# ericehanley/gke-ray-train

Measured on AMD Instinct MI355X. Metric: tokens/sec (whole node) Llama-2-7B fine-tune at 1/2/4/8 MI355X; samples/sec on Wikitext-2, higher is better.
Workload: dtype bf16; 1 GPU; model=llama2-7b, global_batch=8, seq_len=1024, parallelism=dp1, micro_batch=8, grad_accum=1, optimizer=fused AdamW fp32 states, activation_checkpointing=False, optimizer_overlap=True, forced_collectives=False, library_gemms=offline-tuned

## Files before the change

### gke_ray_train_amd/csrc/bindings/ops.cpp

```cpp
#include <climits>
#include <torch/extension.h>

#include <algorithm>
#include <cmath>
#include <c10/hip/HIPStream.h>
#include <c10/core/DeviceGuard.h>

#include "grt_kernels.h"
#include "grt_sdma.h"

namespace {

using at::Tensor;
using c10::optional;

hipStream_t cur_stream(const Tensor& t) {
  return c10::hip::getCurrentHIPStream(t.device().index()).stream();
}

grt::DType dtype_of(const Tensor& t) {
  if (t.scalar_type() == at::kBFloat16) return grt::DType::BF16;
  TORCH_CHECK(t.scalar_type() == at::kFloat, "gke_ray_train_amd kernels support bf16/fp32, got ", t.scalar_type());
  return grt::DType::F32;
}
// ... 1619 lines not shown
  m.def("lora_down", &lora_down, py::arg("x"), py::arg("a"), py::arg("p"), py::arg("seed"), py::arg("offset"),
        py::arg("want_xd"), py::arg("h_out") = py::none(), py::arg("hscale") = 1.0);
  m.def("lora_dx", &lora_dx, py::arg("g"), py::arg("at"), py::arg("dx"), py::arg("p"), py::arg("seed"),
        py::arg("offset"), py::arg("accumulate"), py::arg("dx_in") = py::none(), py::arg("gscale") = 1.0);
  m.def("lora_refresh", &lora_refresh, py::arg("bs"), py::arg("offs"), py::arg("w"), py::arg("wt"), py::arg("col0"),
        py::arg("wt_row0") = -1);
  m.def("lora_g", &lora_g, py::arg("a"), py::arg("bt"), py::arg("c"), py::arg("alpha"), py::arg("accumulate"));
  m.def("lora_g_group", &lora_g_group, py::arg("a"), py::arg("bt"), py::arg("c"), py::arg("alpha"),
        py::arg("accumulate"));
  m.def("lora_tred", &lora_tred, py::arg("a"), py::arg("h"), py::arg("out"), py::arg("alpha"), py::arg("accumulate"),
        py::arg("transpose"));
  m.def("lora_tred_group", &lora_tred_group, py::arg("a"), py::arg("h"), py::arg("out"), py::arg("alpha"),
        py::arg("accumulate"));
  m.def("dropout_bwd_seeded", &dropout_bwd_seeded);
  m.def("ce_fwd", &ce_fwd);
  m.def("ce_bwd", &ce_bwd);
  m.def("sumsq_blocks", &sumsq_blocks);
  m.def("lds_fill", [](int64_t pattern, int64_t device) {
    c10::OptionalDeviceGuard g(c10::Device(c10::DeviceType::CUDA, (c10::DeviceIndex)device));
    grt::lds_fill((uint32_t)pattern, c10::hip::getCurrentHIPStream((c10::DeviceIndex)device).stream());
  }, "test support: fill every CU's LDS with a 32-bit pattern (stale-LDS-read detection)");
  m.def("sumsq", &sumsq);
  m.def("clip_finalize", &clip_finalize);
  m.def("adamw", &adamw, py::arg("p"), py::arg("g"), py::arg("m"), py::arg("v"), py::arg("master"),
        py::arg("hyper"), py::arg("gscale"), py::arg("max_blocks") = 0, py::arg("index_offset") = 0);
  m.def("adamw_t", &adamw_t);
  m.def("adamw8", &adamw8, py::arg("p"), py::arg("g"), py::arg("codes_m"), py::arg("absmax_m"), py::arg("codes_v"),
        py::arg("absmax_v"), py::arg("master"), py::arg("hyper"), py::arg("gscale"), py::arg("max_blocks") = 0,
        py::arg("index_offset") = 0);
  m.def("quantize_blockwise8", &quantize_blockwise8, py::arg("x"), py::arg("codes"), py::arg("absmax"),
        py::arg("signed"));
  m.def("dequantize_blockwise8", &dequantize_blockwise8, py::arg("codes"), py::arg("absmax"), py::arg("out"),
        py::arg("signed"));
  m.def("scale_", &scale_);
  m.def("attn_fwd", &attn_fwd, py::arg("q"), py::arg("k"), py::arg("v"), py::arg("out"), py::arg("scale"),
        py::arg("causal"), py::arg("seqlens_k"), py::arg("dropout_p") = 0.0, py::arg("seed") = 0,
        py::arg("cu_seqlens") = py::none(), py::arg("max_seqlen") = 0, py::arg("o_t") = py::none());
  m.def("attn_bwd", &attn_bwd, py::arg("dout"), py::arg("q"), py::arg("k"), py::arg("v"), py::arg("o"),
        py::arg("lse"), py::arg("dq"), py::arg("dk"), py::arg("dv"), py::arg("scale"), py::arg("causal"),
        py::arg("seqlens_k"), py::arg("dropout_p") = 0.0, py::arg("seed") = 0, py::arg("rope_cos") = py::none(),
        py::arg("rope_sin") = py::none(), py::arg("cu_seqlens") = py::none(), py::arg("max_seqlen") = 0,
        py::arg("dqkv_t") = py::none());
  m.def("rope_attn_fwd_d64", &rope_attn_fwd_d64, py::arg("qkv"), py::arg("cos"), py::arg("sin"), py::arg("o"),
        py::arg("B"), py::arg("S"), py::arg("hq"), py::arg("hkv"), py::arg("scale"), py::arg("causal"),
        py::arg("cu_seqlens") = py::none(), py::arg("max_seqlen") = 0,
        "bf16 head_dim 64: RoPE + flash attention straight from the fused QKV rows (packed with cu_seqlens) -> lse");
  m.def("rope_attn_bwd_d64", &rope_attn_bwd_d64, py::arg("do"), py::arg("qkv"), py::arg("cos"), py::arg("sin"),
        py::arg("o"), py::arg("lse"), py::arg("dqkv"), py::arg("B"), py::arg("S"), py::arg("hq"), py::arg("hkv"),
        py::arg("scale"), py::arg("causal"), py::arg("cu_seqlens") = py::none(), py::arg("max_seqlen") = 0,
        "backward of rope_attn_fwd_d64: un-rotated dQ / dK and dV into the columns of dqkv (every element written)");
  m.def("attn_set_schedule", &grt::attn_set_schedule,
        "bf16 attention causal-pair / XCD-grouped schedule, bit mask: 1 = forward, 2 = dQ, 4 = dK/dV");
  m.def("attn_get_schedule", &grt::attn_get_schedule);
  m.def("attn_set_dkdv_form", &grt::attn_set_dkdv_form, "dK / dV kernel: 1 = 4-wave, 2 = wave-pair (default)");
  m.def("attn_get_dkdv_form", &grt::attn_get_dkdv_form);
  m.def("attn_set_dma_fast", &grt::attn_set_dma_fast, "1 = hoisted LDS-DMA addressing (default), 0 = clamped per tile");
  m.def("ew_set_fast", &grt::ew_set_fast, "1 = single-pass RoPE (D = 128) / SwiGLU kernels (default), 0 = grid-stride kernels");
  m.def("attn_set_skip_dead", &grt::attn_set_skip_dead,
        "1 = forward / dK-dV waves skip the causal tiles they mask entirely (default), 0 = compute them");
  m.def("nf4_quantize", &nf4_quantize);
  m.def("nf4_dequantize", &nf4_dequantize);
  m.def("nf4_dequantize_t", &nf4_dequantize_t);
  m.def("nf4_dequantize_into", &nf4_dequantize_into);
  m.def("rmsnorm_bwd_dx", &rmsnorm_bwd_dx);
  m.def("swiglu_fwd_t", &swiglu_fwd_t);
  m.def("swiglu_bwd_t", &swiglu_bwd_t);
  m.def("transpose_into", &transpose_into);
  m.def("copy_sdma", &copy_sdma);
  m.def("sdma_d2h", &sdma_d2h, py::arg("dst"), py::arg("src"), py::arg("producer_stream") = 0,
        "pinned host <- device on an SDMA engine, ordered on the source's current stream; producer_stream "
        "(a raw stream handle): the stream whose work so far wrote src");
  m.def("sdma_stats", &sdma_stats, "copies / bytes / worker busy seconds / first error of the SDMA copier");
  m.def("sdma_clear_error", [](int64_t device) { grt::sdma_clear_error((int)device); });
  m.def("gemv", &gemv, py::arg("x"), py::arg("w"), py::arg("swiglu") = false);
  m.def("gemv_fused", &gemv_fused, py::arg("x"), py::arg("w"), py::arg("sumsq"), py::arg("slot"),
        py::arg("swiglu") = false, py::arg("g") = py::none(), py::arg("res") = py::none(), py::arg("eps") = 1e-5,
        py::arg("cos") = py::none(), py::arg("sin") = py::none(), py::arg("pos") = py::none(),
        py::arg("kc") = py::none(), py::arg("vc") = py::none(), py::arg("hq") = 0, py::arg("hkv") = 0);
  m.def("nf4_gemv", &nf4_gemv, py::arg("x"), py::arg("qweight"), py::arg("absmax"), py::arg("N"), py::arg("K"),
        py::arg("h") = py::none(), py::arg("lora_b") = py::none(), py::arg("lora_off") = py::none(),
        py::arg("scaling") = 1.0);
  m.def("sample_logits", &sample_logits, py::arg("logits"), py::arg("do_sample") = false, py::arg("temperature") = 1.0,
        py::arg("top_k") = 0, py::arg("top_p") = 1.0, py::arg("seed") = 0, py::arg("counter") = py::none(),
        py::arg("keep_mask") = py::none(), py::arg("finished") = py::none(), py::arg("finish_step") = py::none(),
        py::arg("step") = py::none(), py::arg("next_ids") = py::none(), py::arg("out") = py::none(),
        py::arg("eos_ids") = py::none(), py::arg("pad_id") = py::none(), py::arg("max_steps") = 1);
  m.def("attn_decode", &attn_decode);
  m.def("attn_decode_d64", &attn_decode_d64);
  m.def("attn_decode_d64_partials", &attn_decode_d64_partials,
        "test support: attn_decode_d64 and its per-split (o, max, sum) partial states");
  m.def("embedding_fwd", &embedding_fwd);
  m.def("embedding_bwd", &embedding_bwd);
  m.def("gemm_wgrad", &gemm_wgrad, py::arg("x"), py::arg("y"), py::arg("out"), py::arg("accumulate"),
        py::arg("mode") = 0);
  m.def("gemm_supported", &gemm_supported, py::arg("a"), py::arg("b"), py::arg("out"));
  m.def("gemm_nt", &gemm_nt, py::arg("a"), py::arg("b"), py::arg("out"), py::arg("accumulate") = false,
        py::arg("variant") = 0);
  m.def("gemm_wgrad2", &gemm_wgrad2, py::arg("x"), py::arg("y"), py::arg("out"), py::arg("accumulate") = false);
  m.def("gemm_nn", &gemm_nn, py::arg("a"), py::arg("b"), py::arg("out"), py::arg("accumulate") = false);
  m.def("ipc_alloc", &ipc_alloc);
  m.def("ipc_free", &ipc_free_ptr);
  m.def("ipc_handle", &ipc_handle);
  m.def("ipc_open", &ipc_open);
  m.def("ipc_close", &ipc_close);
  m.def("ipc_allreduce", &ipc_allreduce);
  m.def("ipc_barrier", &ipc_barrier);
  m.def("cu_masked_stream", &cu_masked_stream);
// ... 5 lines not shown
```

### gke_ray_train_amd/csrc/kernels/attention.hip

```cpp
#include <limits.h>
#include <stdlib.h>

#include <type_traits>
#include <utility>

#include "grt_attn_dropout.h"
#include "grt_common.h"
#include "grt_kernels.h"
#include "grt_lds_image.h"
#include "grt_mfma.h"

namespace grt {
namespace {

using namespace lds_image;

constexpr int D = 128;
constexpr int kChunks = D / 8;

__device__ __forceinline__ bf16x8 lds_row_read(const char* base, int row, int ch) {
  return *reinterpret_cast<const bf16x8*>(base + chunk_off(row, ch));
}

constexpr float kLog2e = 1.4426950408889634f;
constexpr float kLn2 = 0.6931471805599453f;

__device__ __forceinline__ float halves_max(float x) {
  const auto r = __builtin_amdgcn_permlane32_swap(__float_as_uint(x), __float_as_uint(x), false, false);
  return fmaxf(__uint_as_float(r[0]), __uint_as_float(r[1]));
}

constexpr float kDeferLog2 = 8.f;

template <class F, int... I>
__device__ __forceinline__ void static_for(F&& f, std::integer_sequence<int, I...>) {
  (f(std::integral_constant<int, I>{}), ...);
}
__device__ __forceinline__ void wait_tiles4(int tiles) {
  if (tiles >= 4) asm volatile("s_waitcnt vmcnt(16)" ::: "memory");
  else if (tiles == 3) asm volatile("s_waitcnt vmcnt(12)" ::: "memory");
  else if (tiles == 2) asm volatile("s_waitcnt vmcnt(8)" ::: "memory");
  else if (tiles == 1) asm volatile("s_waitcnt vmcnt(4)" ::: "memory");
  else asm volatile("s_waitcnt vmcnt(0)" ::: "memory");
}

constexpr int F3M = 128, F3N = 32, F3NT = 256, F3NSLOT = 4;
constexpr int F3IMG = F3N * D * 2;
constexpr int F3SLOT = 2 * F3IMG;

struct QJobs {
  int bh;
  int blk0, blk1;
};
__device__ __forceinline__ QJobs q_jobs(int sched, int nqb, int BH) {
  QJobs j;
  if (sched == 1) {
    const int npair = (nqb + 1) >> 1, nwg = BH * npair;
    const int bid = blockIdx.x, xcd = bid & 7, q8 = nwg >> 3, r8 = nwg & 7;
    const int L = (xcd < r8 ? xcd * (q8 + 1) : r8 * (q8 + 1) + (xcd - r8) * q8) + (bid >> 3);
    j.bh = L / npair;
    const int pr = L % npair;
    j.blk0 = nqb - 1 - pr;
    j.blk1 = pr != nqb - 1 - pr ? pr : -1;
  } else {
    j.bh = blockIdx.x % BH;
    j.blk0 = nqb - 1 - (int)(blockIdx.x / BH);
    j.blk1 = -1;
  }
  return j;
}
__host__ __device__ inline unsigned q_grid(int sched, int nqb, int BH) {
  return (unsigned)(sched == 1 ? BH * ((nqb + 1) / 2) : BH * nqb);
}

template <bool DROP, int NS>
__global__ __launch_bounds__(F3NT, 2) void attn_fwd_kernel(const AttnParams p) {
  __shared__ __attribute__((aligned(16))) char smem[NS * F3SLOT];
  const int tid = threadIdx.x, lane = tid & 63, h = lane >> 5, l32 = lane & 31;
  const int w = __builtin_amdgcn_readfirstlane(tid >> 6);
  const int g = lane >> 4, l16 = lane & 15;
  const int nqb = (p.Sq + F3M - 1) / F3M;
  const int BH = p.B * p.Hq;
  const QJobs jobs = q_jobs(p.sched, nqb, BH);
  const int bh = jobs.bh;
  const int b = bh / p.Hq, hq = bh % p.Hq;
  const int hkv = hq / (p.Hq / p.Hkv);
  GRT_DEVICE_CHECK(b < p.B && hkv < p.Hkv && jobs.blk0 >= 0 && jobs.blk0 < nqb);
  auto run_block = [&](const int qblk) {
  int Sq = p.Sq, Sk = p.Sk;
  int64_t tok0 = 0;
  if (p.cu_seqlens) {
    tok0 = p.cu_seqlens[b];
    Sq = Sk = p.cu_seqlens[b + 1] - (int)tok0;
    if (qblk * F3M >= Sq) return;
  }
  const int sk = p.seqlens_k ? min(Sk, p.seqlens_k[b]) : Sk;
  const int off = Sk - Sq;
  const int q0 = qblk * F3M, qw0 = q0 + w * 32;
  const int myq = qw0 + l32;

  const bf16* Q = (const bf16*)p.q + (int64_t)b * p.q_bs + tok0 * p.q_ss + (int64_t)hq * p.q_hs;
  const bf16* K = (const bf16*)p.k + (int64_t)b * p.k_bs + tok0 * p.k_ss + (int64_t)hkv * p.k_hs;
  const bf16* Vg = (const bf16*)p.v + (int64_t)b * p.v_bs + tok0 * p.v_ss + (int64_t)hkv * p.v_hs;

  bf16x8 qf[D / 16];
#pragma unroll
  for (int ks = 0; ks < D / 16; ++ks) {
    if (myq < Sq) qf[ks] = *reinterpret_cast<const bf16x8*>(Q + (int64_t)myq * p.q_ss + ks * 16 + 8 * h);
    else qf[ks] = bf16x8{};
  }
  const int klim = p.causal ? min(sk - 1, myq + off) : sk - 1;
  const int kmask = p.causal ? min(sk, qw0 + off + 1) : sk;
  const int klast = p.skip_dead && p.causal ? min(sk - 1, qw0 + 31 + off) : INT_MAX;

  int kend = sk;
  if (p.causal) kend = min(kend, q0 + F3M + off);
  const int nt = kend > 0 ? (kend + F3N - 1) / F3N : 0;

  const uint32_t smem0 = lds_addr(smem);
  const int row0 = 8 * w + g, row1 = row0 + 4;
  const int ch0 = l16 ^ swz(row0), ch1 = l16 ^ swz(row1);
  const uint32_t ko0 = (uint32_t)(row0 * p.k_ss + ch0 * 8), ko1 = (uint32_t)(row1 * p.k_ss + ch1 * 8);
  const uint32_t vo0 = (uint32_t)(row0 * p.v_ss + ch0 * 8), vo1 = (uint32_t)(row1 * p.v_ss + ch1 * 8);
  auto dma_tile = [&](int t, uint32_t slot_off) {
    const uint32_t dst = __builtin_amdgcn_readfirstlane(smem0 + slot_off + (uint32_t)(8 * w * 256));
    if (p.dma_fast && (t + 1) * F3N <= Sk) {
// ... 118 lines not shown
    for (; t + UNR <= ntl; t += UNR) static_for([&](auto i_c) { step_i(t, i_c); }, std::make_integer_sequence<int, UNR>{});
    static_for([&](auto i_c) { if (t + decltype(i_c)::value < ntl) step_i(t, i_c); }, std::make_integer_sequence<int, UNR - 1>{});
    for (t = ntl; t < nt; ++t) {
      asm volatile("s_waitcnt lgkmcnt(0)" ::: "memory");
      if (t + 1 < nt) wait_dma(min(nt, t + NS - 1) - (t + 2));
      __builtin_amdgcn_s_barrier();
      if (t + NS - 1 < nt) dma_tile(t + NS - 1, (uint32_t)(((t + NS - 1) % NS) * F3SLOT));
    }
  }
  asm volatile("s_waitcnt vmcnt(0)" ::: "memory");

  const float lt = l + __shfl_xor(l, 32, 64);
  const float inv = lt > 0.f ? 1.f / lt : 0.f;
  bf16* O = (bf16*)p.o + (int64_t)b * p.o_bs + (tok0 + min(myq, Sq - 1)) * p.o_ss + (int64_t)hq * p.o_hs;
#pragma unroll
  for (int db = 0; db < 4; ++db)
#pragma unroll
    for (int gp = 0; gp < 2; ++gp) {
      union { bf16x4 v; uint32_t u[2]; } a, c2;
#pragma unroll
      for (int j = 0; j < 4; ++j) {
        a.v[j] = static_cast<bf16>(o[db][8 * gp + j] * inv);
        c2.v[j] = static_cast<bf16>(o[db][8 * gp + 4 + j] * inv);
      }
      const auto r0 = __builtin_amdgcn_permlane32_swap(a.u[0], c2.u[0], false, false);
      const auto r1 = __builtin_amdgcn_permlane32_swap(a.u[1], c2.u[1], false, false);
      if (myq < Sq) {
        *reinterpret_cast<uint4*>(O + db * 32 + 16 * gp + 8 * h) = make_uint4(r0[0], r1[0], r0[1], r1[1]);
        if (p.o_t != nullptr) {
          bf16* ot = static_cast<bf16*>(p.o_t) + (int64_t)(hq * D) * p.ot_ld + (p.cu_seqlens ? 0 : (int64_t)b * p.Sq) +
                     tok0 + myq;
          const int d0 = db * 32 + 8 * (2 * gp) + 4 * h, d1 = db * 32 + 8 * (2 * gp + 1) + 4 * h;
#pragma unroll
          for (int j = 0; j < 4; ++j) {
            ot[(int64_t)(d0 + j) * p.ot_ld] = a.v[j];
            ot[(int64_t)(d1 + j) * p.ot_ld] = c2.v[j];
          }
        }
      }
    }
  if (myq < Sq) {
    if (h == 0 && p.lse)
      p.lse[((int64_t)b * p.Hq + hq) * p.Sq + myq] = lt > 0.f ? (m + __log2f(lt)) * kLn2 : INFINITY;
  }
  };
  run_block(jobs.blk0);
  if (jobs.blk1 >= 0) {
    asm volatile("s_waitcnt lgkmcnt(0)" ::: "memory");
    __builtin_amdgcn_s_barrier();
    run_block(jobs.blk1);
  }
}

__host__ __device__ inline int sq_pad(int Sq) { return (Sq + 31) / 32 * 32; }

__global__ __launch_bounds__(256) void attn_bwd_pre_kernel(const AttnBwdParams p) {
  const int l16 = threadIdx.x & 15;
  const int Sqp = sq_pad(p.f.Sq);
  const int64_t row = (int64_t)blockIdx.x * 16 + (threadIdx.x >> 4);
  const int64_t nrows = (int64_t)p.f.B * p.f.Hq * Sqp;
  if (row >= nrows) return;
  const int q = (int)(row % Sqp);
  const int64_t bh = row / Sqp;
  float acc = 0.f;
  const int hq = (int)(bh % p.f.Hq), b = (int)(bh / p.f.Hq);
  int Sq = p.f.Sq;
  int64_t tok0 = 0;
  if (p.f.cu_seqlens) {
    tok0 = p.f.cu_seqlens[b];
    Sq = p.f.cu_seqlens[b + 1] - (int)tok0;
  }
  if (q < Sq) {
    const bf16* O = (const bf16*)p.f.o + (int64_t)b * p.f.o_bs + (int64_t)hq * p.f.o_hs + (tok0 + q) * p.f.o_ss;
    const bf16* dO = (const bf16*)p.dout + (int64_t)b * p.do_bs + (int64_t)hq * p.do_hs + (tok0 + q) * p.do_ss;
    float a[8], g[8];
    load16(O + l16 * 8, a);
    load16(dO + l16 * 8, g);
#pragma unroll
    for (int k = 0; k < 8; ++k) acc += a[k] * g[k];
  }
#pragma unroll
  for (int o = 8; o >= 1; o >>= 1) acc += __shfl_xor(acc, o, 16);
  if (l16 == 0) {
    float* lse2 = p.delta + nrows;
    p.delta[row] = acc;
    lse2[row] = q < Sq ? p.f.lse[bh * p.f.Sq + q] * kLog2e : INFINITY;
  }
}


struct TCopy {
  bf16* p;
  int64_t ld;
};
__device__ __forceinline__ void st_t(const TCopy& tc, int d, const bf16x4& v) {
  if (tc.p != nullptr) {
#pragma unroll
    for (int j = 0; j < 4; ++j) tc.p[(int64_t)(d + j) * tc.ld] = v[j];
  }
}
__device__ __forceinline__ TCopy tcopy(const AttnBwdParams& P, int row0, int head, int64_t tok) {
  if (P.dqkv_t == nullptr) return TCopy{nullptr, 0};
  return TCopy{static_cast<bf16*>(P.dqkv_t) + (int64_t)(row0 + head * D) * P.t_ld + tok, P.t_ld};
}

__device__ __forceinline__ void store_unrotated(const f32x16 (&acc)[4], float scale, const float* __restrict__ cr,
                                                const float* __restrict__ sr, bf16* dst, int h,
                                                const TCopy& tc = TCopy{nullptr, 0}) {
#pragma unroll
  for (int db = 0; db < 2; ++db)
#pragma unroll
    for (int gg = 0; gg < 4; ++gg) {
      const int d = db * 32 + 8 * gg + 4 * h;
      const f32x4 c = *reinterpret_cast<const f32x4*>(cr + d);
      const f32x4 sn = *reinterpret_cast<const f32x4*>(sr + d);
      bf16x4 lo, hi;
#pragma unroll
      for (int j = 0; j < 4; ++j) {
        const float x1 = acc[db][4 * gg + j] * scale, x2 = acc[db + 2][4 * gg + j] * scale;
        lo[j] = static_cast<bf16>(x1 * c[j] + x2 * sn[j]);
        hi[j] = static_cast<bf16>(x2 * c[j] - x1 * sn[j]);
      }
      *reinterpret_cast<bf16x4*>(dst + d) = lo;
      *reinterpret_cast<bf16x4*>(dst + d + D / 2) = hi;
      st_t(tc, d, lo);
      st_t(tc, d + D / 2, hi);
    }
}

constexpr int K2N = 128, K2M = 32, K2NT = 256, K2NSLOT = 4;
constexpr int K2IMG = K2M * D * 2;
constexpr int K2SLOT = 2 * K2IMG + 4 * 1024;

template <bool DROP>
__global__ __launch_bounds__(K2NT, 1) void attn_bwd_dkdv_kernel(const AttnBwdParams P) {
  const AttnParams& p = P.f;
  __shared__ __attribute__((aligned(16))) char smem[K2NSLOT * K2SLOT];
  const int tid = threadIdx.x, lane = tid & 63, h = lane >> 5, l32 = lane & 31;
  const int w = __builtin_amdgcn_readfirstlane(tid >> 6);
  const int g = lane >> 4, l16 = lane & 15;
  const int BHk = p.B * p.Hkv;
  const int nkb = (p.Sk + K2N - 1) / K2N;
  QJobs jobs;
  if (p.sched == 1) {
    jobs = q_jobs(1, nkb, BHk);
  } else {
    jobs.bh = blockIdx.x % BHk;
    jobs.blk0 = (int)(blockIdx.x / BHk);
    jobs.blk1 = -1;
  }
  const int bhk = jobs.bh;
  const int b = bhk / p.Hkv, hkv = bhk % p.Hkv;
  const int grp = p.Hq / p.Hkv;
  auto run_block = [&](const int kblk) {
  int Sq = p.Sq, Sk = p.Sk;
  int64_t tok0 = 0;
  if (p.cu_seqlens) {
    tok0 = p.cu_seqlens[b];
    Sq = Sk = p.cu_seqlens[b + 1] - (int)tok0;
    if (kblk * K2N >= Sk) return;
  }
  GRT_DEVICE_CHECK(grp * p.Hkv == p.Hq && kblk * K2N < Sk);
  const int sk = p.seqlens_k ? min(Sk, p.seqlens_k[b]) : Sk;
  const int off = Sk - Sq;
  const int k0 = kblk * K2N, kw0 = k0 + w * 32, mykey = kw0 + l32;
  const float c = p.scale * kLog2e;
  const int Sqp = sq_pad(p.Sq);
  const float* lse2 = P.delta + (int64_t)p.B * p.Hq * Sqp;

  const bf16* K = (const bf16*)p.k + (int64_t)b * p.k_bs + tok0 * p.k_ss + (int64_t)hkv * p.k_hs;
  const bf16* Vg = (const bf16*)p.v + (int64_t)b * p.v_bs + tok0 * p.v_ss + (int64_t)hkv * p.v_hs;
  bf16x8 kf[D / 16], vf[D / 16];
#pragma unroll
  for (int ks = 0; ks < D / 16; ++ks) {
    if (mykey < sk) {
      kf[ks] = *reinterpret_cast<const bf16x8*>(K + (int64_t)mykey * p.k_ss + ks * 16 + 8 * h);
      vf[ks] = *reinterpret_cast<const bf16x8*>(Vg + (int64_t)mykey * p.v_ss + ks * 16 + 8 * h);
    } else {
      kf[ks] = bf16x8{};
      vf[ks] = bf16x8{};
    }
// ... 363 lines not shown
      bf16x8 fq[D / 16];
#pragma unroll
      for (int ks = 0; ks < D / 16; ++ks) fq[ks] = lds_row_read(qi, l32, 2 * ks + h);
#pragma unroll
      for (int ks = 0; ks < D / 16; ++ks) s = mfma32(fq[ks], kv[ks], s);
      __builtin_amdgcn_sched_barrier(0);
      float* xo = xbase + (t & 1) * (K3X / 4);
#pragma unroll
      for (int q = 0; q < 4; ++q) {
        const f32x4 ls = *reinterpret_cast<const f32x4*>(st + 8 * q + 4 * h);
        f32x4 pv;
#pragma unroll
        for (int j = 0; j < 4; ++j) pv[j] = fast_exp2(fmaf(s[4 * q + j], c, -ls[j]));
        *reinterpret_cast<f32x4*>(xo + (q * 64 + lane) * 4) = pv;
#pragma unroll
        for (int j = 0; j < 4; ++j) s[4 * q + j] = pv[j];
      }
      const bf16x8 pb0 = pack8(s, 0), pb1 = pack8(s, 8);
      __builtin_amdgcn_sched_barrier(0);
#pragma unroll
      for (int stp = 0; stp < 2; ++stp) {
        const int kk = 16 * stp + 4 * h;
#pragma unroll
        for (int db = 0; db < 4; ++db) {
          const int c0 = db * 32 + (g & 1) * 16;
          const bf16x8 a = cat(tr_read(qi + K3IMG, kk, c0, l16), tr_read(qi + K3IMG, kk + 8, c0, l16));
          acc[db] = mfma32(a, stp ? pb1 : pb0, acc[db]);
        }
      }
     }
    } else {
      if (t > 0 && !dead_p) finish(t - 1, smem + ((SL + K3NS - 1) % K3NS) * K3SLOT);
      __builtin_amdgcn_sched_barrier(0);
      if (!dead_c) {
        bf16x8 fd[D / 16];
#pragma unroll
        for (int ks = 0; ks < D / 16; ++ks) fd[ks] = lds_row_read(qi + K3IMG, l32, 2 * ks + h);
        dpc = f32x16{};
#pragma unroll
        for (int ks = 0; ks < D / 16; ++ks) dpc = mfma32(fd[ks], kv[ks], dpc);
      }
    }
    prv_h = cur_h;
    prv_q = cur_q;
    advance(cur_h, cur_q);
  };

  if (total > 0) {
    const int pre = min(total, K3PD);
    for (int j = 0; j < pre; ++j) {
      dma_tile(hkv * grp + dma_h, dma_q, (uint32_t)(j * K3SLOT));
      advance(dma_h, dma_q);
    }
    using I0 = std::integral_constant<int, 0>;
    using I1 = std::integral_constant<int, 1>;
    using I2 = std::integral_constant<int, 2>;
    using I3 = std::integral_constant<int, 3>;
    using I4 = std::integral_constant<int, 4>;
    int t = 0;
    for (; t + K3NS <= total; t += K3NS) {
      step(t, I0{});
      step(t + 1, I1{});
      step(t + 2, I2{});
      step(t + 3, I3{});
      step(t + 4, I4{});
    }
    if (t < total) step(t, I0{});
    if (t + 1 < total) step(t + 1, I1{});
    if (t + 2 < total) step(t + 2, I2{});
    if (t + 3 < total) step(t + 3, I3{});
    asm volatile("s_waitcnt lgkmcnt(0)" ::: "memory");
    __builtin_amdgcn_s_barrier();
    if constexpr (!SW) {
      if (prv_q + K3M > dead_q) finish(total - 1, smem + ((total - 1) % K3NS) * K3SLOT);
    }
  }
  asm volatile("s_waitcnt vmcnt(0)" ::: "memory");

  if (mykey < Sk) {
    const int64_t tokg = (p.cu_seqlens ? 0 : (int64_t)b * p.Sk) + tok0 + mykey;
    if constexpr (SW) {
      bf16* dV = (bf16*)P.dv + (int64_t)b * P.dv_bs + (int64_t)hkv * P.dv_hs + (tok0 + mykey) * P.dv_ss;
      const TCopy tv = tcopy(P, P.t_row_v, hkv, tokg);
#pragma unroll
      for (int db = 0; db < 4; ++db)
#pragma unroll
        for (int gg = 0; gg < 4; ++gg) {
          bf16x4 v;
#pragma unroll
          for (int j = 0; j < 4; ++j) v[j] = static_cast<bf16>(acc[db][4 * gg + j]);
          *reinterpret_cast<bf16x4*>(dV + db * 32 + 8 * gg + 4 * h) = v;
          st_t(tv, db * 32 + 8 * gg + 4 * h, v);
        }
    } else {
      bf16* dK = (bf16*)P.dk + (int64_t)b * P.dk_bs + (int64_t)hkv * P.dk_hs + (tok0 + mykey) * P.dk_ss;
      const TCopy tk = tcopy(P, P.t_row_k, hkv, tokg);
      if (P.rope_cos) {
        store_unrotated(acc, p.scale, P.rope_cos + (int64_t)mykey * (D / 2), P.rope_sin + (int64_t)mykey * (D / 2), dK, h,
                        tk);
      } else {
#pragma unroll
        for (int db = 0; db < 4; ++db)
#pragma unroll
          for (int gg = 0; gg < 4; ++gg) {
            bf16x4 a;
#pragma unroll
// ... 160 lines not shown
  };

  if (nt > 0) {
    const int pre = min(nt, Q2NSLOT - 1);
    for (int t = 0; t < pre; ++t) dma_tile(t, (uint32_t)(t * Q2SLOT));
    wait_dma(pre - 1);
    __builtin_amdgcn_s_barrier();
    f32x16 sA, dpA, sB, dpB;
    sdp(0, I0{}, sA, dpA);
    int t = 0;
    for (; t + Q2NSLOT <= nt; t += Q2NSLOT) {
      step(t, I0{}, sA, dpA, sB, dpB);
      step(t + 1, std::integral_constant<int, 1>{}, sB, dpB, sA, dpA);
      step(t + 2, std::integral_constant<int, 2>{}, sA, dpA, sB, dpB);
      step(t + 3, std::integral_constant<int, 3>{}, sB, dpB, sA, dpA);
    }
    if (t < nt) step(t, I0{}, sA, dpA, sB, dpB);
    if (t + 1 < nt) step(t + 1, std::integral_constant<int, 1>{}, sB, dpB, sA, dpA);
    if (t + 2 < nt) step(t + 2, std::integral_constant<int, 2>{}, sA, dpA, sB, dpB);
  }
  asm volatile("s_waitcnt vmcnt(0)" ::: "memory");

  if (qok) {
    bf16* dQ = (bf16*)P.dq + (int64_t)b * P.dq_bs + (int64_t)hq * P.dq_hs + (tok0 + myq) * P.dq_ss;
    const TCopy tq = tcopy(P, P.t_row_q, hq, (p.cu_seqlens ? 0 : (int64_t)b * p.Sq) + tok0 + myq);
    if (P.rope_cos) {
      store_unrotated(dq, p.scale, P.rope_cos + (int64_t)myq * (D / 2), P.rope_sin + (int64_t)myq * (D / 2), dQ, h, tq);
    } else {
#pragma unroll
      for (int db = 0; db < 4; ++db)
#pragma unroll
        for (int gg = 0; gg < 4; ++gg) {
          bf16x4 v;
#pragma unroll
          for (int j = 0; j < 4; ++j) v[j] = static_cast<bf16>(dq[db][4 * gg + j] * p.scale);
          *reinterpret_cast<bf16x4*>(dQ + db * 32 + 8 * gg + 4 * h) = v;
          st_t(tq, db * 32 + 8 * gg + 4 * h, v);
        }
    }
  }
  };
  run_block(jobs.blk0);
  if (jobs.blk1 >= 0) {
    asm volatile("s_waitcnt lgkmcnt(0)" ::: "memory");
    __builtin_amdgcn_s_barrier();
    run_block(jobs.blk1);
  }
}

}

namespace {
int g_sched = 7;
int g_dkdv = 2;
int g_skip_dead = -1;
int skip_dead_now() {
  if (g_skip_dead < 0) {
    const char* e = getenv("GRT_ATTN_SKIP");
    g_skip_dead = e && atoi(e) == 0 ? 0 : 1;
  }
  return g_skip_dead;
}
int g_dma_fast = 1;
int dma_fast_for(const AttnParams& p, int64_t do_ss) {
  const int64_t lim = (int64_t)1 << 24;
  return g_dma_fast && p.q_ss < lim && p.k_ss < lim && p.v_ss < lim && do_ss < lim && p.q_ss >= 0 &&
         p.k_ss >= 0 && p.v_ss >= 0 && do_ss >= 0;
}
}

static int cu_count() {
  static const int n = [] {
    int d = 0, c = 256;
    hipGetDevice(&d);
    hipDeviceGetAttribute(&c, hipDeviceAttributeMultiprocessorCount, d);
    return c > 0 ? c : 256;
  }();
  return n;
}
static int pair_if_fills(int want, int nblk, int groups, int per_cu) {
  return want && (int64_t)groups * ((nblk + 1) / 2) >= (int64_t)cu_count() * per_cu ? 1 : 0;
}

void attn_set_schedule(int s) { g_sched = s; }
void attn_set_dkdv_form(int f) { g_dkdv = f == 1 ? 1 : 2; }
int attn_get_dkdv_form() { return g_dkdv; }
void attn_set_dma_fast(int on) { g_dma_fast = on ? 1 : 0; }
void attn_set_skip_dead(int on) { g_skip_dead = on ? 1 : 0; }
int attn_get_schedule() { return g_sched; }

static int sched_for(const AttnParams& p, int bit) { return p.cu_seqlens ? 0 : (g_sched >> bit) & 1; }

void attn_fwd(const AttnParams& p0, hipStream_t s) {
  AttnParams p = p0;
  p.dma_fast = dma_fast_for(p, 0);
  p.skip_dead = skip_dead_now();
  const int nqb = (p.Sq + F3M - 1) / F3M;
  p.sched = pair_if_fills(sched_for(p, 0), nqb, p.B * p.Hq, 2);
  const dim3 grid(q_grid(p.sched, nqb, p.B * p.Hq));
  if (p.drop_thresh) hipLaunchKernelGGL((attn_fwd_kernel<true, F3NSLOT>), grid, dim3(F3NT), 0, s, p);
  else hipLaunchKernelGGL((attn_fwd_kernel<false, F3NSLOT>), grid, dim3(F3NT), 0, s, p);
}

int64_t attn_bwd_workspace_floats(int B, int Hq, int Sq, int Dh) {
  (void)Dh;
  return 2 * (int64_t)B * Hq * sq_pad(Sq);
}

void attn_bwd(const AttnBwdParams& p0, hipStream_t s) {
  AttnBwdParams p = p0;
  p.f.dma_fast = dma_fast_for(p.f, p.do_ss);
  p.f.skip_dead = skip_dead_now();
  const int64_t rows = (int64_t)p.f.B * p.f.Hq * sq_pad(p.f.Sq);
  hipLaunchKernelGGL(attn_bwd_pre_kernel, dim3((unsigned)((rows + 15) / 16)), dim3(256), 0, s, p);
  const int nkb = (p.f.Sk + K2N - 1) / K2N;
  const int nqb = (p.f.Sq + Q2M - 1) / Q2M;
  AttnBwdParams pk = p, pq = p;
  pk.f.sched = pair_if_fills(sched_for(p.f, 2), nkb, p.f.B * p.f.Hkv, 1);
  pq.f.sched = pair_if_fills(sched_for(p.f, 1), nqb, p.f.B * p.f.Hq, 2);
  const dim3 g1(q_grid(pk.f.sched, nkb, p.f.B * p.f.Hkv)), g2(q_grid(pq.f.sched, nqb, p.f.B * p.f.Hq));
  static_assert(K3N == K2N, "both dK / dV forms take 128-key blocks (same grid)");
  if (p.f.drop_thresh) {
    hipLaunchKernelGGL(attn_bwd_dkdv_kernel<true>, g1, dim3(K2NT), 0, s, pk);
    hipLaunchKernelGGL(attn_bwd_dq_kernel<true>, g2, dim3(Q2NT), 0, s, pq);
  } else {
    if (g_dkdv == 2) hipLaunchKernelGGL(attn_bwd_dkdv2_kernel, g1, dim3(K3NT), 0, s, pk);
    else hipLaunchKernelGGL(attn_bwd_dkdv_kernel<false>, g1, dim3(K2NT), 0, s, pk);
    hipLaunchKernelGGL(attn_bwd_dq_kernel<false>, g2, dim3(Q2NT), 0, s, pq);
  }
}

}
```

Baseline: 28390 tokens/s.

## Add 256-key dK/dV attention backward kernel with 64 keys per wave pair

Adds a new dK/dV backward kernel in which each 512-thread workgroup handles 256 keys, split into four wave pairs of 64 keys. One wave of each pair computes the P/dV path and the other computes the dP/dK path, with a five-slot LDS pipeline for Q/dO tiles. The launcher picks it by default when there is no GQA, no packing, and the grid covers the CUs. This amortizes Q/dO tile loads over more keys per workgroup. The cost is one workgroup per CU and more registers; it also moves shared helpers into a header and adds a waitcnt in the existing kernel prologue.

```diff
diff --git a/gke_ray_train_amd/csrc/bindings/ops.cpp b/gke_ray_train_amd/csrc/bindings/ops.cpp
--- a/gke_ray_train_amd/csrc/bindings/ops.cpp
+++ b/gke_ray_train_amd/csrc/bindings/ops.cpp
@@ -1695,7 +1695,7 @@
   m.def("attn_set_schedule", &grt::attn_set_schedule,
         "bf16 attention causal-pair / XCD-grouped schedule, bit mask: 1 = forward, 2 = dQ, 4 = dK/dV");
   m.def("attn_get_schedule", &grt::attn_get_schedule);
-  m.def("attn_set_dkdv_form", &grt::attn_set_dkdv_form, "dK / dV kernel: 1 = 4-wave, 2 = wave-pair (default)");
+  m.def("attn_set_dkdv_form", &grt::attn_set_dkdv_form, "dK / dV kernel: 0 = chosen per launch (default), 1 = 4-wave, 2 = wave-pair, 32 keys per pair, 3 = wave-pair, 64 keys per pair");
   m.def("attn_get_dkdv_form", &grt::attn_get_dkdv_form);
   m.def("attn_set_dma_fast", &grt::attn_set_dma_fast, "1 = hoisted LDS-DMA addressing (default), 0 = clamped per tile");
   m.def("ew_set_fast", &grt::ew_set_fast, "1 = single-pass RoPE (D = 128) / SwiGLU kernels (default), 0 = grid-stride kernels");
diff --git a/gke_ray_train_amd/csrc/include/grt_attn_bwd.h b/gke_ray_train_amd/csrc/include/grt_attn_bwd.h
--- /dev/null
+++ b/gke_ray_train_amd/csrc/include/grt_attn_bwd.h
@@ -0,0 +1,90 @@
+#pragma once
+#include <hip/hip_runtime.h>
+
+#include "grt_common.h"
+#include "grt_kernels.h"
+#include "grt_lds_image.h"
+#include "grt_mfma.h"
+
+namespace grt {
+namespace attn128 {
+
+constexpr int D = 128;
+constexpr float kLog2e = 1.4426950408889634f;
+
+__device__ __forceinline__ bf16x8 lds_row_read(const char* base, int row, int ch) {
+  return *reinterpret_cast<const bf16x8*>(base + lds_image::chunk_off(row, ch));
+}
+
+struct QJobs {
+  int bh;
+  int blk0, blk1;
+};
+__device__ __forceinline__ QJobs q_jobs(int sched, int nqb, int BH) {
+  QJobs j;
+  if (sched == 1) {
+    const int npair = (nqb + 1) >> 1, nwg = BH * npair;
+    const int bid = blockIdx.x, xcd = bid & 7, q8 = nwg >> 3, r8 = nwg & 7;
+    const int L = (xcd < r8 ? xcd * (q8 + 1) : r8 * (q8 + 1) + (xcd - r8) * q8) + (bid >> 3);
+    j.bh = L / npair;
+    const int pr = L % npair;
+    j.blk0 = nqb - 1 - pr;
+    j.blk1 = pr != nqb - 1 - pr ? pr : -1;
+  } else {
+    j.bh = blockIdx.x % BH;
+    j.blk0 = nqb - 1 - (int)(blockIdx.x / BH);
+    j.blk1 = -1;
+  }
+  return j;
+}
+__host__ __device__ inline unsigned q_grid(int sched, int nqb, int BH) {
+  return (unsigned)(sched == 1 ? BH * ((nqb + 1) / 2) : BH * nqb);
+}
+
+__host__ __device__ inline int sq_pad(int Sq) { return (Sq + 31) / 32 * 32; }
+
+struct TCopy {
+  bf16* p;
+  int64_t ld;
+};
+__device__ __forceinline__ void st_t(const TCopy& tc, int d, const bf16x4& v) {
+  if (tc.p != nullptr) {
+#pragma unroll
+    for (int j = 0; j < 4; ++j) tc.p[(int64_t)(d + j) * tc.ld] = v[j];
+  }
+}
+__device__ __forceinline__ TCopy tcopy(const AttnBwdParams& P, int row0, int head, int64_t tok) {
+  if (P.dqkv_t == nullptr) return TCopy{nullptr, 0};
+  return TCopy{static_cast<bf16*>(P.dqkv_t) + (int64_t)(row0 + head * D) * P.t_ld + tok, P.t_ld};
+}
+
+__device__ __forceinline__ void store_unrotated(const f32x16 (&acc)[4], float scale, const float* __restrict__ cr,
+                                                const float* __restrict__ sr, bf16* dst, int h,
+                                                const TCopy& tc = TCopy{nullptr, 0}) {
+#pragma unroll
+  for (int db = 0; db < 2; ++db)
+#pragma unroll
+    for (int gg = 0; gg < 4; ++gg) {
+      const int d = db * 32 + 8 * gg + 4 * h;
+      const f32x4 c = *reinterpret_cast<const f32x4*>(cr + d);
+      const f32x4 sn = *reinterpret_cast<const f32x4*>(sr + d);
+      bf16x4 lo, hi;
+#pragma unroll
+      for (int j = 0; j < 4; ++j) {
+        const float x1 = acc[db][4 * gg + j] * scale, x2 = acc[db + 2][4 * gg + j] * scale;
+        lo[j] = static_cast<bf16>(x1 * c[j] + x2 * sn[j]);
+        hi[j] = static_cast<bf16>(x2 * c[j] - x1 * sn[j]);
+      }
+      *reinterpret_cast<bf16x4*>(dst + d) = lo;
+      *reinterpret_cast<bf16x4*>(dst + d + D / 2) = hi;
+      st_t(tc, d, lo);
+      st_t(tc, d + D / 2, hi);
+    }
+}
+
+}
+
+constexpr int kDkdv64Keys = 256;
+void attn_bwd_dkdv64_launch(const AttnBwdParams& p, unsigned grid, hipStream_t s);
+
+}
diff --git a/gke_ray_train_amd/csrc/kernels/attention.hip b/gke_ray_train_amd/csrc/kernels/attention.hip
--- a/gke_ray_train_amd/csrc/kernels/attention.hip
+++ b/gke_ray_train_amd/csrc/kernels/attention.hip
@@ -4,6 +4,7 @@
 #include <type_traits>
 #include <utility>
 
+#include "grt_attn_bwd.h"
 #include "grt_attn_dropout.h"
 #include "grt_common.h"
 #include "grt_kernels.h"
@@ -14,15 +15,10 @@
 namespace {
 
 using namespace lds_image;
-
-constexpr int D = 128;
+using namespace attn128;
+
 constexpr int kChunks = D / 8;
 
-__device__ __forceinline__ bf16x8 lds_row_read(const char* base, int row, int ch) {
-  return *reinterpret_cast<const bf16x8*>(base + chunk_off(row, ch));
-}
-
-constexpr float kLog2e = 1.4426950408889634f;
 constexpr float kLn2 = 0.6931471805599453f;
 
 __device__ __forceinline__ float halves_max(float x) {
@@ -47,31 +43,6 @@
 constexpr int F3M = 128, F3N = 32, F3NT = 256, F3NSLOT = 4;
 constexpr int F3IMG = F3N * D * 2;
 constexpr int F3SLOT = 2 * F3IMG;
-
-struct QJobs {
-  int bh;
-  int blk0, blk1;
-};
-__device__ __forceinline__ QJobs q_jobs(int sched, int nqb, int BH) {
-  QJobs j;
-  if (sched == 1) {
-    const int npair = (nqb + 1) >> 1, nwg = BH * npair;
-    const int bid = blockIdx.x, xcd = bid & 7, q8 = nwg >> 3, r8 = nwg & 7;
-    const int L = (xcd < r8 ? xcd * (q8 + 1) : r8 * (q8 + 1) + (xcd - r8) * q8) + (bid >> 3);
-    j.bh = L / npair;
-    const int pr = L % npair;
-    j.blk0 = nqb - 1 - pr;
-    j.blk1 = pr != nqb - 1 - pr ? pr : -1;
-  } else {
-    j.bh = blockIdx.x % BH;
-    j.blk0 = nqb - 1 - (int)(blockIdx.x / BH);
-    j.blk1 = -1;
-  }
-  return j;
-}
-__host__ __device__ inline unsigned q_grid(int sched, int nqb, int BH) {
-  return (unsigned)(sched == 1 ? BH * ((nqb + 1) / 2) : BH * nqb);
-}
 
 template <bool DROP, int NS>
 __global__ __launch_bounds__(F3NT, 2) void attn_fwd_kernel(const AttnParams p) {
@@ -296,8 +267,6 @@
   }
 }
 
-__host__ __device__ inline int sq_pad(int Sq) { return (Sq + 31) / 32 * 32; }
-
 __global__ __launch_bounds__(256) void attn_bwd_pre_kernel(const AttnBwdParams p) {
   const int l16 = threadIdx.x & 15;
   const int Sqp = sq_pad(p.f.Sq);
@@ -332,45 +301,6 @@
   }
 }
 
-
-struct TCopy {
-  bf16* p;
-  int64_t ld;
-};
-__device__ __forceinline__ void st_t(const TCopy& tc, int d, const bf16x4& v) {
-  if (tc.p != nullptr) {
-#pragma unroll
-    for (int j = 0; j < 4; ++j) tc.p[(int64_t)(d + j) * tc.ld] = v[j];
-  }
-}
-__device__ __forceinline__ TCopy tcopy(const AttnBwdParams& P, int row0, int head, int64_t tok) {
-  if (P.dqkv_t == nullptr) return TCopy{nullptr, 0};
-  return TCopy{static_cast<bf16*>(P.dqkv_t) + (int64_t)(row0 + head * D) * P.t_ld + tok, P.t_ld};
-}
-
-__device__ __forceinline__ void store_unrotated(const f32x16 (&acc)[4], float scale, const float* __restrict__ cr,
-                                                const float* __restrict__ sr, bf16* dst, int h,
-                                                const TCopy& tc = TCopy{nullptr, 0}) {
-#pragma unroll
-  for (int db = 0; db < 2; ++db)
-#pragma unroll
-    for (int gg = 0; gg < 4; ++gg) {
-      const int d = db * 32 + 8 * gg + 4 * h;
-      const f32x4 c = *reinterpret_cast<const f32x4*>(cr + d);
-      const f32x4 sn = *reinterpret_cast<const f32x4*>(sr + d);
-      bf16x4 lo, hi;
-#pragma unroll
-      for (int j = 0; j < 4; ++j) {
-        const float x1 = acc[db][4 * gg + j] * scale, x2 = acc[db + 2][4 * gg + j] * scale;
-        lo[j] = static_cast<bf16>(x1 * c[j] + x2 * sn[j]);
-        hi[j] = static_cast<bf16>(x2 * c[j] - x1 * sn[j]);
-      }
-      *reinterpret_cast<bf16x4*>(dst + d) = lo;
-      *reinterpret_cast<bf16x4*>(dst + d + D / 2) = hi;
-      st_t(tc, d, lo);
-      st_t(tc, d + D / 2, hi);
-    }
-}
 
 constexpr int K2N = 128, K2M = 32, K2NT = 256, K2NSLOT = 4;
 constexpr int K2IMG = K2M * D * 2;
@@ -840,6 +770,7 @@
       dma_tile(hkv * grp + dma_h, dma_q, (uint32_t)(j * K3SLOT));
       advance(dma_h, dma_q);
     }
+    __builtin_amdgcn_s_waitcnt(0x0F70);
     using I0 = std::integral_constant<int, 0>;
     using I1 = std::integral_constant<int, 1>;
     using I2 = std::integral_constant<int, 2>;
@@ -1106,7 +1037,7 @@
 
 namespace {
 int g_sched = 7;
-int g_dkdv = 2;
+int g_dkdv = 0;
 int g_skip_dead = -1;
 int skip_dead_now() {
   if (g_skip_dead < 0) {
@@ -1137,7 +1068,7 @@
 }
 
 void attn_set_schedule(int s) { g_sched = s; }
-void attn_set_dkdv_form(int f) { g_dkdv = f == 1 ? 1 : 2; }
+void attn_set_dkdv_form(int f) { g_dkdv = f >= 0 && f <= 3 ? f : 2; }
 int attn_get_dkdv_form() { return g_dkdv; }
 void attn_set_dma_fast(int on) { g_dma_fast = on ? 1 : 0; }
 void attn_set_skip_dead(int on) { g_skip_dead = on ? 1 : 0; }
@@ -1178,8 +1109,18 @@
     hipLaunchKernelGGL(attn_bwd_dkdv_kernel<true>, g1, dim3(K2NT), 0, s, pk);
     hipLaunchKernelGGL(attn_bwd_dq_kernel<true>, g2, dim3(Q2NT), 0, s, pq);
   } else {
-    if (g_dkdv == 2) hipLaunchKernelGGL(attn_bwd_dkdv2_kernel, g1, dim3(K3NT), 0, s, pk);
-    else hipLaunchKernelGGL(attn_bwd_dkdv_kernel<false>, g1, dim3(K2NT), 0, s, pk);
+    const int nkb64 = (p.f.Sk + kDkdv64Keys - 1) / kDkdv64Keys;
+    const int sched64 = pair_if_fills(sched_for(p.f, 2), nkb64, p.f.B * p.f.Hkv, 1);
+    const unsigned grid64 = q_grid(sched64, nkb64, p.f.B * p.f.Hkv);
+    const bool take64 = g_dkdv == 3 || (g_dkdv == 0 && !p.f.cu_seqlens && p.f.Hq == p.f.Hkv && (int)grid64 >= cu_count());
+    if (take64) {
+      pk.f.sched = sched64;
+      attn_bwd_dkdv64_launch(pk, grid64, s);
+    } else if (g_dkdv != 1) {
+      hipLaunchKernelGGL(attn_bwd_dkdv2_kernel, g1, dim3(K3NT), 0, s, pk);
+    } else {
+      hipLaunchKernelGGL(attn_bwd_dkdv_kernel<false>, g1, dim3(K2NT), 0, s, pk);
+    }
     hipLaunchKernelGGL(attn_bwd_dq_kernel<false>, g2, dim3(Q2NT), 0, s, pq);
   }
 }
diff --git a/gke_ray_train_amd/csrc/kernels/attention_dkdv64.hip b/gke_ray_train_amd/csrc/kernels/attention_dkdv64.hip
--- /dev/null
+++ b/gke_ray_train_amd/csrc/kernels/attention_dkdv64.hip
@@ -0,0 +1,351 @@
+#include <limits.h>
+
+#include <type_traits>
+#include <utility>
+
+#include "grt_attn_bwd.h"
+#include "grt_common.h"
+#include "grt_kernels.h"
+#include "grt_lds_image.h"
+#include "grt_mfma.h"
+
+namespace grt {
+namespace {
+
+using namespace lds_image;
+using namespace attn128;
+
+constexpr int K4N = kDkdv64Keys, K4M = 32, K4NT = 512, K4NS = 5, K4PD = K4NS - 2;
+constexpr int K4IMG = K4M * D * 2;
+constexpr int K4SLOT = 2 * K4IMG + 1024;
+constexpr int K4XS = 64 * 16 * 4;
+constexpr int K4X = 4 * 2 * K4XS;
+constexpr int K4LDS = K4NS * K4SLOT + 2 * K4X;
+static_assert(K4N == 4 * 64 && K4LDS <= 160 * 1024, "4 pairs of 64 keys; one workgroup per CU");
+
+__global__ __launch_bounds__(K4NT, 1) void attn_bwd_dkdv64_kernel(const AttnBwdParams P) {
+  const AttnParams& p = P.f;
+  __shared__ __attribute__((aligned(16))) char smem[K4LDS];
+  const int w = __builtin_amdgcn_readfirstlane((int)threadIdx.x >> 6);
+  const int pr = w & 3;
+  const bool swave = w < 4;
+  auto lane_now = []() __attribute__((always_inline)) {
+    int x;
+    asm volatile("v_mbcnt_lo_u32_b32 %0, -1, 0\n\tv_mbcnt_hi_u32_b32 %0, -1, %0" : "=v"(x));
+    return x;
+  };
+  const int BHk = p.B * p.Hkv;
+  const int nkb = (p.Sk + K4N - 1) / K4N;
+  QJobs jobs;
+  if (p.sched == 1) {
+    jobs = q_jobs(1, nkb, BHk);
+  } else {
+    jobs.bh = blockIdx.x % BHk;
+    jobs.blk0 = (int)(blockIdx.x / BHk);
+    jobs.blk1 = -1;
+  }
+  const int bhk = jobs.bh;
+  const int b = bhk / p.Hkv, hkv = bhk % p.Hkv;
+  const int grp = p.Hq / p.Hkv;
+  auto run_block = [&](const int kblk, auto role_c) __attribute__((always_inline)) {
+  constexpr bool SW = decltype(role_c)::value;
+  int Sq = p.Sq, Sk = p.Sk;
+  int64_t tok0 = 0;
+  if (p.cu_seqlens) {
+    tok0 = p.cu_seqlens[b];
+    Sq = Sk = p.cu_seqlens[b + 1] - (int)tok0;
+    if (kblk * K4N >= Sk) return;
+  }
+  GRT_DEVICE_CHECK(grp * p.Hkv == p.Hq && kblk * K4N < Sk);
+  const int sk = p.seqlens_k ? min(Sk, p.seqlens_k[b]) : Sk;
+  const int off = Sk - Sq;
+  const int k0 = kblk * K4N, kw0 = k0 + pr * 64;
+  const float c = p.scale * kLog2e;
+  const int Sqp = sq_pad(p.Sq);
+
+  const bf16* KV = SW ? (const bf16*)p.k + (int64_t)b * p.k_bs + tok0 * p.k_ss + (int64_t)hkv * p.k_hs
+                         : (const bf16*)p.v + (int64_t)b * p.v_bs + tok0 * p.v_ss + (int64_t)hkv * p.v_hs;
+  const int64_t kv_ss = SW ? p.k_ss : p.v_ss;
+  bf16x8 kv[2][D / 16];
+  {
+    const int lane = lane_now(), h = lane >> 5;
+#pragma unroll
+    for (int j = 0; j < 2; ++j) {
+      const int key = kw0 + 32 * j + (lane & 31);
+#pragma unroll
+      for (int ks = 0; ks < D / 16; ++ks)
+        kv[j][ks] = key < sk ? *reinterpret_cast<const bf16x8*>(KV + (int64_t)key * kv_ss + ks * 16 + 8 * h) : bf16x8{};
+    }
+  }
+  f32x16 acc[2][4];
+#pragma unroll
+  for (int j = 0; j < 2; ++j)
+#pragma unroll
+    for (int i = 0; i < 4; ++i) acc[j][i] = f32x16{};
+
+  int qstart = p.causal ? max(0, k0 - off) : 0;
+  qstart = (qstart / K4M) * K4M;
+  const int nqt = qstart < Sq ? (Sq - qstart + K4M - 1) / K4M : 0;
+  const int total = (k0 < sk) ? nqt * grp : 0;
+  int qmask[2];
+#pragma unroll
+  for (int j = 0; j < 2; ++j) qmask[j] = (k0 + K4N > sk) ? INT_MAX : (p.causal ? kw0 + 32 * j + 31 - off : INT_MIN);
+  const int dead_q = p.skip_dead && p.causal ? kw0 - off : INT_MIN;
+
+  const uint32_t smem0 = lds_addr(smem);
+  auto dma_tile = [&](int hq, int qt, uint32_t slot_off) __attribute__((always_inline)) {
+    const bf16* Q = (const bf16*)p.q + (int64_t)b * p.q_bs + tok0 * p.q_ss + (int64_t)hq * p.q_hs;
+    const bf16* dO = (const bf16*)P.dout + (int64_t)b * P.do_bs + tok0 * P.do_ss + (int64_t)hq * P.do_hs;
+    const uint32_t dst = __builtin_amdgcn_readfirstlane(smem0 + slot_off + (uint32_t)(4 * w * 256));
+    const int lane = lane_now(), l16 = lane & 15;
+    const int row = 4 * w + (lane >> 4), ch = l16 ^ swz(row);
+    if (p.dma_fast && qt + K4M <= Sq) {
+      const uint32_t qo = (uint32_t)(row * (int)p.q_ss + ch * 8), oo = (uint32_t)(row * (int)P.do_ss + ch * 8);
+      lds_dma16_keep_m0(Q + (int64_t)qt * p.q_ss + qo, dst);
+      lds_dma16_keep_m0(dO + (int64_t)qt * P.do_ss + oo, dst + K4IMG);
+    } else {
+      const int64_t qr = min(qt + row, Sq - 1);
+      lds_dma16_keep_m0(Q + qr * p.q_ss + ch * 8, dst);
+      lds_dma16_keep_m0(dO + qr * P.do_ss + ch * 8, dst + K4IMG);
+    }
+    if (SW && w == 0) {
+      const int64_t st_lane = (l16 < 8 ? (int64_t)p.B * p.Hq * Sqp : 0) + 4 * (l16 & 7);
+      const int64_t ri = ((int64_t)b * p.Hq + hq) * Sqp + qt;
+      lds_dma16_keep_m0(P.delta + st_lane + ri, __builtin_amdgcn_readfirstlane(smem0 + slot_off + (uint32_t)(2 * K4IMG)));
+    }
+  };
+  auto wait_dma = [&](int pending_tiles) __attribute__((always_inline)) {
+    if (SW && w == 0) {
+      if (pending_tiles >= 2) asm volatile("s_waitcnt vmcnt(6)" ::: "memory");
+      else if (pending_tiles == 1) asm volatile("s_waitcnt vmcnt(3)" ::: "memory");
+      else asm volatile("s_waitcnt vmcnt(0)" ::: "memory");
+    } else {
+      if (pending_tiles >= 2) asm volatile("s_waitcnt vmcnt(4)" ::: "memory");
+      else if (pending_tiles == 1) asm volatile("s_waitcnt vmcnt(2)" ::: "memory");
+      else asm volatile("s_waitcnt vmcnt(0)" ::: "memory");
+    }
+  };
+  float* const xbase = reinterpret_cast<float*>(smem + K4NS * K4SLOT) + pr * (2 * K4XS / 4);
+
+  int cur_h = 0, cur_q = qstart, prv_h = 0, prv_q = qstart, dma_h = 0, dma_q = qstart;
+  auto advance = [&](int& hh, int& qq) __attribute__((always_inline)) {
+    qq += K4M;
+    if (qq >= Sq) { qq = qstart; ++hh; }
+  };
+  f32x16 dpc[2] = {f32x16{}, f32x16{}};
+
+  auto row_base = [&]() __attribute__((always_inline)) {
+    const int lane = lane_now();
+    return (uint32_t)chunk_off(lane & 31, lane >> 5);
+  };
+  auto tr_base = [&]() __attribute__((always_inline)) {
+    const int lane = lane_now(), h = lane >> 5, g = lane >> 4, l16 = lane & 15;
+    const int tcol = (g & 1) * 16 + 4 * (l16 & 3);
+    return (uint32_t)(chunk_off(4 * h + (l16 >> 2), tcol >> 3) + 8 * ((tcol >> 2) & 1));
+  };
+  auto tr_at = [](const char* a) __attribute__((always_inline)) {
+    return __builtin_amdgcn_ds_read_tr16_b64_v4bf16((lds_bf16x4*)a);
+  };
+
+  auto accumulate = [&](const char* img, const bf16x8 (&bb)[2][2]) __attribute__((always_inline)) {
+#pragma unroll
+    for (int stp = 0; stp < 2; ++stp) {
+      const uint32_t tb = tr_base();
+#pragma unroll
+      for (int db = 0; db < 4; ++db) {
+        const uint32_t o = tb ^ (uint32_t)(db << 6);
+        const bf16x8 a = cat(tr_at(img + o + 4096 * stp), tr_at(img + (o ^ 32u) + 2048 + 4096 * stp));
+        acc[0][db] = mfma32(a, bb[0][stp], acc[0][db]);
+        acc[1][db] = mfma32(a, bb[1][stp], acc[1][db]);
+      }
+    }
+  };
+  auto rows_x_kv = [&](const char* img, f32x16 (&x)[2]) __attribute__((always_inline)) {
+#pragma unroll
+    for (int qu = 0; qu < 4; ++qu) {
+      const uint32_t rb = row_base();
+      bf16x8 f[2];
+#pragma unroll
+      for (int i = 0; i < 2; ++i) f[i] = *reinterpret_cast<const bf16x8*>(img + (rb ^ (uint32_t)((2 * qu + i) << 5)));
+#pragma unroll
+      for (int i = 0; i < 2; ++i) {
+        x[0] = mfma32(f[i], kv[0][2 * qu + i], x[0]);
+        x[1] = mfma32(f[i], kv[1][2 * qu + i], x[1]);
+      }
+      __builtin_amdgcn_sched_barrier(0);
+    }
+  };
+
+  auto finish = [&](int tp, const char* pi) __attribute__((always_inline)) {
+    const float* st = reinterpret_cast<const float*>(pi + 2 * K4IMG);
+    const float* xi = xbase + (tp & 1) * (K4X / 4);
+    bf16x8 sb[2][2];
+#pragma unroll
+    for (int j = 0; j < 2; ++j)
+#pragma unroll
+      for (int stp = 0; stp < 2; ++stp) {
+        const int lane = lane_now(), h = lane >> 5;
+#pragma unroll
+        for (int q = 2 * stp; q < 2 * stp + 2; ++q) {
+          const f32x4 pv = *reinterpret_cast<const f32x4*>(xi + j * (K4XS / 4) + (q * 64 + lane) * 4);
+          const f32x4 de = *reinterpret_cast<const f32x4*>(st + 32 + 8 * q + 4 * h);
+#pragma unroll
+          for (int e = 0; e < 4; ++e)
+            sb[j][stp][4 * (q - 2 * stp) + e] = static_cast<bf16>(pv[e] * (dpc[j][4 * q + e] - de[e]));
+        }
+        __builtin_amdgcn_sched_barrier(0);
+      }
+    accumulate(pi, sb);
+  };
+
+  auto step = [&](int t, auto slot_c) __attribute__((always_inline)) {
+    constexpr int SL = decltype(slot_c)::value;
+    asm volatile("s_waitcnt lgkmcnt(0)" ::: "memory");
+    wait_dma(min(total - 1, t + K4PD - 1) - t);
+    __builtin_amdgcn_s_barrier();
+    if (t + K4PD < total) {
+      dma_tile(hkv * grp + dma_h, dma_q, (uint32_t)(((SL + K4PD) % K4NS) * K4SLOT));
+      advance(dma_h, dma_q);
+    }
+    const char* qi = smem + SL * K4SLOT;
+    const bool dead_c = cur_q + K4M <= dead_q, dead_p = prv_q + K4M <= dead_q;
+    if constexpr (SW) {
+     if (!dead_c) {
+      const float* st = reinterpret_cast<const float*>(qi + 2 * K4IMG);
+      f32x16 s[2];
+#pragma unroll
+      for (int j = 0; j < 2; ++j) {
+        s[j] = f32x16{};
+        if (cur_q < qmask[j]) {
+          const int lane = lane_now(), h = lane >> 5, key = kw0 + 32 * j + (lane & 31);
+          const int qlim = key < sk ? (p.causal ? key - off : INT_MIN) : INT_MAX;
+#pragma unroll
+          for (int r = 0; r < 16; ++r) s[j][r] = cur_q + acc_row(r, h) >= qlim ? 0.f : -INFINITY;
+        }
+      }
+      rows_x_kv(qi, s);
+      float* xo = xbase + (t & 1) * (K4X / 4);
+      bf16x8 pb[2][2];
+#pragma unroll
+      for (int j = 0; j < 2; ++j) {
+        const int lane = lane_now(), h = lane >> 5;
+#pragma unroll
+        for (int q = 0; q < 4; ++q) {
+          const f32x4 ls = *reinterpret_cast<const f32x4*>(st + 8 * q + 4 * h);
+          f32x4 pv;
+#pragma unroll
+          for (int e = 0; e < 4; ++e) pv[e] = fast_exp2(fmaf(s[j][4 * q + e], c, -ls[e]));
+          *reinterpret_cast<f32x4*>(xo + j * (K4XS / 4) + (q * 64 + lane) * 4) = pv;
+#pragma unroll
+          for (int e = 0; e < 4; ++e) s[j][4 * q + e] = pv[e];
+        }
+        pb[j][0] = pack8(s[j], 0);
+        pb[j][1] = pack8(s[j], 8);
+        __builtin_amdgcn_sched_barrier(0);
+      }
+      accumulate(qi + K4IMG, pb);
+     }
+    } else {
+      if (t > 0 && !dead_p) finish(t - 1, smem + ((SL + K4NS - 1) % K4NS) * K4SLOT);
+      __builtin_amdgcn_sched_barrier(0);
+      if (!dead_c) {
+        dpc[0] = f32x16{};
+        dpc[1] = f32x16{};
+        rows_x_kv(qi + K4IMG, dpc);
+      }
+    }
+    prv_h = cur_h;
+    prv_q = cur_q;
+    advance(cur_h, cur_q);
+  };
+
+  if (total > 0) {
+    const int pre = min(total, K4PD);
+    for (int j = 0; j < pre; ++j) {
+      dma_tile(hkv * grp + dma_h, dma_q, (uint32_t)(j * K4SLOT));
+      advance(dma_h, dma_q);
+    }
+    __builtin_amdgcn_s_waitcnt(0x0F70);
+    using I0 = std::integral_constant<int, 0>;
+    using I1 = std::integral_constant<int, 1>;
+    using I2 = std::integral_constant<int, 2>;
+    using I3 = std::integral_constant<int, 3>;
+    using I4 = std::integral_constant<int, 4>;
+    int t = 0;
+    for (; t + K4NS <= total; t += K4NS) {
+      step(t, I0{});
+      step(t + 1, I1{});
+      step(t + 2, I2{});
+      step(t + 3, I3{});
+      step(t + 4, I4{});
+    }
+    if (t < total) step(t, I0{});
+    if (t + 1 < total) step(t + 1, I1{});
+    if (t + 2 < total) step(t + 2, I2{});
+    if (t + 3 < total) step(t + 3, I3{});
+    asm volatile("s_waitcnt lgkmcnt(0)" ::: "memory");
+    __builtin_amdgcn_s_barrier();
+    if constexpr (!SW) {
+      if (prv_q + K4M > dead_q) finish(total - 1, smem + ((total - 1) % K4NS) * K4SLOT);
+    }
+  }
+  asm volatile("s_waitcnt vmcnt(0)" ::: "memory");
+
+#pragma unroll
+  for (int j = 0; j < 2; ++j) {
+    const int lane = lane_now(), h = lane >> 5, key = kw0 + 32 * j + (lane & 31);
+    if (key >= Sk) continue;
+    const int64_t tokg = (p.cu_seqlens ? 0 : (int64_t)b * p.Sk) + tok0 + key;
+    if constexpr (SW) {
+      bf16* dV = (bf16*)P.dv + (int64_t)b * P.dv_bs + (int64_t)hkv * P.dv_hs + (tok0 + key) * P.dv_ss;
+      const TCopy tv = tcopy(P, P.t_row_v, hkv, tokg);
+#pragma unroll
+      for (int db = 0; db < 4; ++db)
+#pragma unroll
+        for (int gg = 0; gg < 4; ++gg) {
+          bf16x4 v;
+#pragma unroll
+          for (int e = 0; e < 4; ++e) v[e] = static_cast<bf16>(acc[j][db][4 * gg + e]);
+          *reinterpret_cast<bf16x4*>(dV + db * 32 + 8 * gg + 4 * h) = v;
+          st_t(tv, db * 32 + 8 * gg + 4 * h, v);
+        }
+    } else {
+      bf16* dK = (bf16*)P.dk + (int64_t)b * P.dk_bs + (int64_t)hkv * P.dk_hs + (tok0 + key) * P.dk_ss;
+      const TCopy tk = tcopy(P, P.t_row_k, hkv, tokg);
+      if (P.rope_cos) {
+        store_unrotated(acc[j], p.scale, P.rope_cos + (int64_t)key * (D / 2), P.rope_sin + (int64_t)key * (D / 2), dK,
+                        h, tk);
+      } else {
+#pragma unroll
+        for (int db = 0; db < 4; ++db)
+#pragma unroll
+          for (int gg = 0; gg < 4; ++gg) {
+            bf16x4 a;
+#pragma unroll
+            for (int e = 0; e < 4; ++e) a[e] = static_cast<bf16>(acc[j][db][4 * gg + e] * p.scale);
+            *reinterpret_cast<bf16x4*>(dK + db * 32 + 8 * gg + 4 * h) = a;
+            st_t(tk, db * 32 + 8 * gg + 4 * h, a);
+          }
+      }
+    }
+  }
+  };
+  auto run_role = [&](auto role_c) __attribute__((always_inline)) {
+    run_block(jobs.blk0, role_c);
+    if (jobs.blk1 >= 0) {
+      asm volatile("s_waitcnt lgkmcnt(0)" ::: "memory");
+      __builtin_amdgcn_s_barrier();
+      run_block(jobs.blk1, role_c);
+    }
+  };
+  if (swave) run_role(std::true_type{});
+  else run_role(std::false_type{});
+}
+
+}
+
+void attn_bwd_dkdv64_launch(const AttnBwdParams& p, unsigned grid, hipStream_t s) {
+  hipLaunchKernelGGL(attn_bwd_dkdv64_kernel, dim3(grid), dim3(K4NT), 0, s, p);
+}
+
+}
```

New measurement: 28390 tokens/s (median of 2 runs). Within noise of the previous version (-0.0%).
